# PaddlePaddle/Paddle3D

Measured on NVIDIA H100. Metric: CenterPoint frames/sec @300k pts, 0.075m voxel (0.1m voxel: geometry_01m), 1440x1440x40 grid, higher is better.
Workload: dtype f16x3 (fp16 hi/lo' pairs, f32 accumulation)

## Files before the change

paddle3d_b200/csrc/dense_conv_f16.cu:

```cuda
#include <cuda.h>
#include <cuda_fp16.h>

#include "h16.cuh"
#include "p3d_b200.h"
#include "tc_common.cuh"

namespace p3d {
namespace dcf {

using namespace tc;

constexpr int kTW = 8, kTH = 16;
constexpr int kPitch = kTW + 2;
constexpr int kMaxA = 6, kMaxB = 12;
constexpr int kSmemBudget = (227 - 6) * 1024;
constexpr int kDenseThreads = 384;
constexpr uint32_t kConsumerWarps = 8;
constexpr uint32_t kEpiThreads = 96;

struct Params {
  int B, H, W, Cin;
  int taps, kw, stride, pad;
  int up;
  int oH, oW;
  int tiles_x, tiles_y, n_ntiles;
  int cout;
  int out_H, out_W;
  int out_C, out_c0;
  int relu;
  const uint8_t *packed_w;
  const float *scale, *shift;
  uint8_t *out_h16;
  float *out_nchw;
  int32_t *status;
};

template <int N, int MT, bool HALO>
struct Cfg {
  static constexpr int A_ROWS = HALO ? kPitch * (kTH * MT + 2) : kM * MT;
  static constexpr int A_BYTES = ((A_ROWS * 128 + 1023) / 1024) * 1024;
  static constexpr int B_BYTES = 128 * N;
  static constexpr int B_BLK = 64 * N;
  static constexpr int SP = N + 8;
  static constexpr int STG_WG = MT * 64 * SP;
  static constexpr int STG_BYTES = 2 * STG_WG * 4;
  static constexpr int AVAIL = kSmemBudget - STG_BYTES;
  static constexpr int NA_TAP_RAW = AVAIL / (A_BYTES + B_BYTES);
  static constexpr int NA = HALO ? 2 : (NA_TAP_RAW > kMaxA ? kMaxA : NA_TAP_RAW);
  static constexpr int BUDGET = AVAIL - NA * A_BYTES;
  static constexpr int NB_RAW = BUDGET / B_BYTES;
  static constexpr int NB = NB_RAW > kMaxB ? kMaxB : NB_RAW;
  static constexpr int ACC = MT * N;
  static constexpr int SPU = HALO ? 9 : 1;
  static constexpr int P_REGS = 88, C_REGS = 208;
  static_assert(128 * P_REGS + 256 * C_REGS <= kDenseThreads * 168, "register split");
  static_assert(N == 64 || N == 128, "N tile: 64 or 128");
  static_assert(MT == 1 || MT == 2, "one or two M tiles");
  static_assert(MT * N <= 128, "accumulators: at most 128 registers per thread");
  static_assert(NB >= 3, "weight ring too shallow");
  static_assert(NA >= 2 && NA <= kMaxA, "activation ring depth");
};

__device__ __forceinline__ void tma_tile4d(uint32_t dst, const CUtensorMap *map, int c, int x, int y, int b, uint32_t bar) {
  asm volatile(
      "cp.async.bulk.tensor.4d.shared::cluster.global.tile.mbarrier::complete_tx::bytes [%0], [%1, {%2, %3, %4, %5}], [%6];" ::
          "r"(dst),
      "l"(reinterpret_cast<uint64_t>(map)), "r"(c), "r"(x), "r"(y), "r"(b), "r"(bar)
      : "memory");
}
struct Item {
  int nt, tap0, tx0, ty0, b;
};

enum TraceField {
  kTrItems, kTrCycles,
  kTrAFull, kTrBFull = kTrAFull + 2,
  kTrMma = kTrBFull + 2,
  kTrEpi = kTrMma + 2,
  kTrStageFree = kTrEpi + 2,
  kTrAEmpty = kTrStageFree + 2, kTrBEmpty,
  kTrEwWait, kTrEwBusy,
  kTrFields
};
#ifdef P3D_DENSE_TRACE
constexpr int kTrMaxCtas = 1024;
__device__ unsigned long long g_dense_trace[kTrMaxCtas][kTrFields];
struct Trace {
  unsigned long long sum[kTrFields] = {};
  __device__ __forceinline__ long long now() const { return clock64(); }
  __device__ __forceinline__ void add(int f, long long t0) { sum[f] += static_cast<unsigned long long>(clock64() - t0); }
  __device__ __forceinline__ void count(int f, unsigned long long v) { sum[f] += v; }
  __device__ void flush(int cw) const {
#pragma unroll
    for (int f = 0; f < kTrFields; ++f) {
      const int dst = f >= kTrAFull && f < kTrAEmpty ? f + cw : f;
      if (sum[f]) atomicAdd(&g_dense_trace[blockIdx.x % kTrMaxCtas][dst], sum[f]);
    }
  }
};
#else
struct Trace {
  __device__ __forceinline__ long long now() const { return 0; }
  __device__ __forceinline__ void add(int, long long) {}
  __device__ __forceinline__ void count(int, unsigned long long) {}
  __device__ __forceinline__ void flush(int) const {}
};
#endif
__device__ __forceinline__ Item decode(long long idx, const Params &p, int th) {
  Item it;
  long long q = blockIdx.x + idx * gridDim.x;
  it.nt = static_cast<int>(q % p.n_ntiles);
  q /= p.n_ntiles;
  it.tap0 = 0;
  if (p.up > 1) {
    const int up2 = p.up * p.up;
    it.tap0 = static_cast<int>(q % up2);
    q /= up2;
  }
  it.tx0 = static_cast<int>(q % p.tiles_x) * kTW;
  q /= p.tiles_x;
  it.ty0 = static_cast<int>(q % p.tiles_y) * th;
  it.b = static_cast<int>(q / p.tiles_y);
  return it;
}

template <int N, int MT>
__device__ __forceinline__ void epilogue_warps(const Params &p, const float *stg, unsigned long long *staged,
                                               unsigned long long *freed, long long n_items, int th, int et) {
  constexpr int SP = N + 8, ROWS = MT * 64;
  const int ew = et >> 5, lane = et & 31;
  bool ovf = false;
  Trace tr;
  for (long long idx = 0; idx < n_items; ++idx) {
    const Item im = decode(idx, p, th);
    const int dy = p.up > 1 ? im.tap0 / p.up : 0, dx = p.up > 1 ? im.tap0 % p.up : 0;
    for (int c = 0; c < 2; ++c) {
      long long t0 = tr.now();
      mbar_wait(smem_u32(staged + c), static_cast<uint32_t>(idx & 1));
      tr.add(kTrEwWait, t0);
      t0 = tr.now();
      const float *st = stg + c * ROWS * SP;
      auto pixel = [&](int r, int &Y, int &X) {
        const int m = c * 64 + (r & 63), iy = im.ty0 + (r >> 6) * kTH + m / kTW, ix = im.tx0 + m % kTW;
        Y = iy * p.up + dy;
        X = ix * p.up + dx;
        return iy < p.oH && ix < p.oW;
      };
      if (p.out_h16) {
        const int r4 = lane >> 3, c4 = (lane & 7) * 4;
        for (int q = 0; q < N / 32; ++q) {
          const int col = q * 32 + c4, ch = im.nt * N + col, oc = p.out_c0 + ch;
          if (ch >= p.cout) continue;
          float sc[4], sh[4];
#pragma unroll
          for (int e = 0; e < 4; ++e) {
            sc[e] = p.scale ? __ldg(p.scale + ch + e) : 1.0f;
            sh[e] = p.shift ? __ldg(p.shift + ch + e) : 0.0f;
          }
#pragma unroll 2
          for (int rq = ew; rq < ROWS / 4; rq += 3) {
            const int r = rq * 4 + r4;
            int Y, X;
            if (!pixel(r, Y, X)) continue;
            const float4 o4 = *reinterpret_cast<const float4 *>(st + r * SP + col);
            float v[4] = {o4.x, o4.y, o4.z, o4.w};
#pragma unroll
            for (int e = 0; e < 4; ++e) {
              v[e] = fmaf(v[e], sc[e], sh[e]);
              if (p.relu) v[e] = fmaxf(v[e], 0.f);
            }
            __half2 h01, l01, h23, l23;
            split_h16x2(v[0], v[1], h01, l01, ovf);
            split_h16x2(v[2], v[3], h23, l23, ovf);
            uint8_t *op = p.out_h16 + ((static_cast<size_t>(im.b) * p.out_H + Y) * p.out_W + X) * (4 * static_cast<size_t>(p.out_C)) +
                          (oc / 32) * 128 + (oc % 32) * 2;
            *reinterpret_cast<uint2 *>(op) = make_uint2(*reinterpret_cast<const uint32_t *>(&h01), *reinterpret_cast<const uint32_t *>(&h23));
            *reinterpret_cast<uint2 *>(op + 64) = make_uint2(*reinterpret_cast<const uint32_t *>(&l01), *reinterpret_cast<const uint32_t *>(&l23));
          }
        }
      }
      if (p.out_nchw) {
        const int px = lane & 7, cc = lane >> 3;
        for (int u = ew; u < (ROWS / 8) * (N / 4); u += 3) {
          const int r = (u % (ROWS / 8)) * 8 + px, col = (u / (ROWS / 8)) * 4 + cc, ch = im.nt * N + col;
          int Y, X;
          if (ch >= p.cout || !pixel(r, Y, X)) continue;
          const float sc = p.scale ? __ldg(p.scale + ch) : 1.0f, sh = p.shift ? __ldg(p.shift + ch) : 0.0f;
          float v = fmaf(st[r * SP + col], sc, sh);
          if (p.relu) v = fmaxf(v, 0.f);
          p.out_nchw[((static_cast<size_t>(im.b) * p.cout + ch) * p.out_H + Y) * p.out_W + X] = v;
        }
      }
      mbar_arrive(smem_u32(freed + c));
      tr.add(kTrEwBusy, t0);
    }
  }
  if (ovf && p.status) atomicOr(p.status, 1);
  if (et == 0) tr.flush(0);
}

template <int N, int MT, bool HALO>
__global__ void __launch_bounds__(kDenseThreads, 1)
    dense_conv_f16_kernel(const __grid_constant__ CUtensorMap in_map, const Params p) {
  using C = Cfg<N, MT, HALO>;
  constexpr int TH = kTH * MT;
  constexpr int H = N / 2;
  asm volatile("griddepcontrol.launch_dependents;" ::: "memory");
  asm volatile("griddepcontrol.wait;" ::: "memory");
  const int up2 = p.up * p.up;
  const long long n_total = static_cast<long long>(p.B) * p.tiles_y * p.tiles_x * p.n_ntiles * (p.up > 1 ? up2 : 1);
  if (static_cast<long long>(blockIdx.x) >= n_total) return;
  const long long n_items = (n_total - blockIdx.x + gridDim.x - 1) / gridDim.x;

  extern __shared__ __align__(1024) uint8_t smem_raw[];
  uint8_t *smem = reinterpret_cast<uint8_t *>((reinterpret_cast<uintptr_t>(smem_raw) + 1023) & ~uintptr_t(1023));
  __shared__ __align__(8) unsigned long long s_bar[2 * kMaxA + 2 * kMaxB + 4];
  constexpr int kAF = 0, kAE = kMaxA, kBF = 2 * kMaxA, kBE = 2 * kMaxA + kMaxB, kSS = 2 * kMaxA + 2 * kMaxB, kSF = kSS + 2;

  const int tid = threadIdx.x, wg = tid >> 7, wtid = tid & 127;
  if (tid == 0) {
    for (int s = 0; s < C::NA; ++s) {
      mbar_init(smem_u32(&s_bar[kAF + s]), 1);
      mbar_init(smem_u32(&s_bar[kAE + s]), kConsumerWarps);
    }
    for (int s = 0; s < C::NB; ++s) {
      mbar_init(smem_u32(&s_bar[kBF + s]), 1);
      mbar_init(smem_u32(&s_bar[kBE + s]), kConsumerWarps);
    }
    for (int c = 0; c < 2; ++c) {
      mbar_init(smem_u32(&s_bar[kSS + c]), 128);
      mbar_init(smem_u32(&s_bar[kSF + c]), kEpiThreads);
    }
    fence_mbar_init();
  }
  __syncthreads();
  const uint32_t a_ring = smem_u32(smem);
  const uint32_t b_ring = a_ring + C::NA * C::A_BYTES;
  float *const stg = reinterpret_cast<float *>(smem + C::NA * C::A_BYTES + C::NB * C::B_BYTES);
  const int G = p.Cin / 32;
  const int taps_item = p.up > 1 ? 1 : p.taps;
  const int units_item = HALO ? G : taps_item * G;

  if (wg == 0) {
    asm volatile("setmaxnreg.dec.sync.aligned.u32 %0;" ::"n"(C::P_REGS));
    if (tid >= 32) {
      epilogue_warps<N, MT>(p, stg, s_bar + kSS, s_bar + kSF, n_items, TH, tid - 32);
      return;
    }
    if (tid != 0) return;
    uint32_t a_slot = 0, a_ph = 0, b_slot = 0, b_ph = 0;
    Trace tr;
    for (long long idx = 0; idx < n_items; ++idx) {
      const Item im = decode(idx, p, TH);
      const uint8_t *w_tile = p.packed_w + static_cast<size_t>(im.nt) * p.taps * (p.Cin / 16) * C::B_BLK;
      int dy = 0, dx = 0;
      for (int tu = 0; tu < (HALO ? 1 : taps_item); ++tu) {
        const int tap = p.up > 1 ? im.tap0 : tu;
        for (int g = 0; g < G; ++g) {
          const uint32_t abar = smem_u32(&s_bar[kAF + a_slot]), a_dst = a_ring + a_slot * C::A_BYTES;
          const long long t0 = tr.now();
          mbar_wait(smem_u32(&s_bar[kAE + a_slot]), a_ph ^ 1u);
          tr.add(kTrAEmpty, t0);
          mbar_arrive_expect_tx(abar, static_cast<uint32_t>(C::A_ROWS * 128));
          if (HALO) {
            tma_tile4d(a_dst, &in_map, g * 64, im.tx0 - 1, im.ty0 - 1, im.b, abar);
          } else {
            const int x = im.tx0 * p.stride - p.pad + dx, y = im.ty0 * p.stride - p.pad + dy;
            tma_tile4d(a_dst, &in_map, g * 64, x, y, im.b, abar);
          }
          if (++a_slot == C::NA) a_slot = 0, a_ph ^= 1u;
          for (int t = 0; t < C::SPU; ++t) {
            const uint32_t bbar = smem_u32(&s_bar[kBF + b_slot]);
            const long long t1 = tr.now();
            mbar_wait(smem_u32(&s_bar[kBE + b_slot]), b_ph ^ 1u);
            tr.add(kTrBEmpty, t1);
            mbar_arrive_expect_tx(bbar, static_cast<uint32_t>(C::B_BYTES));
            bulk_g2s(b_ring + b_slot * C::B_BYTES, w_tile + (static_cast<size_t>(HALO ? t : tap) * (p.Cin / 16) + 2 * g) * C::B_BLK,
                     static_cast<uint32_t>(C::B_BYTES), bbar);
            if (++b_slot == C::NB) b_slot = 0, b_ph ^= 1u;
          }
        }
        if (++dx == p.kw) dx = 0, ++dy;
      }
    }
    tr.flush(0);
    return;
  }

  asm volatile("setmaxnreg.inc.sync.aligned.u32 %0;" ::"n"(C::C_REGS));
  const int cw = wg - 1;
  const bool warp_leader = (tid & 31) == 0;
  auto release = [&](int base, uint32_t slot) {
    if (warp_leader) mbar_arrive(smem_u32(&s_bar[base + slot]));
  };
  uint32_t a_slot = 0, a_ph = 0, b_slot = 0, b_ph = 0;
  float acc[C::ACC];
  Trace tr;
  const long long t_start = tr.now();
  for (long long idx = 0; idx < n_items; ++idx) {
#pragma unroll
    for (int i = 0; i < C::ACC; ++i) acc[i] = 0.f;
    uint32_t prev_b = 0;
    int prev_a = -1;
    bool pending = false;
    for (int ua = 0; ua < units_item; ++ua) {
      long long t0 = tr.now();
      mbar_wait(smem_u32(&s_bar[kAF + a_slot]), a_ph);
      tr.add(kTrAFull, t0);
      const uint32_t a_base = a_ring + a_slot * C::A_BYTES;
      for (int t = 0; t < C::SPU; ++t) {
        t0 = tr.now();
        mbar_wait(smem_u32(&s_bar[kBF + b_slot]), b_ph);
        tr.add(kTrBFull, t0);
        const uint32_t b_base = b_ring + b_slot * C::B_BYTES;
        wg_fence();
#pragma unroll
        for (int kb = 0; kb < 2; ++kb) {
          const uint32_t bk = b_base + static_cast<uint32_t>(kb * C::B_BLK);
          const uint64_t dbh = smem_desc(bk, 2 * N * 16, 128), dbl = smem_desc(bk + N * 16, 2 * N * 16, 128);
#pragma unroll
          for (int mt = 0; mt < MT; ++mt) {
            uint32_t a0, sbo;
            if (HALO) {
              a0 = a_base + static_cast<uint32_t>(((mt * kTH + cw * 8 + t / 3) * kPitch + t % 3) * 128);
              sbo = kPitch * 128;
            } else {
              a0 = a_base + static_cast<uint32_t>((mt * kM + cw * 64) * 128);
              sbo = 1024;
            }
            const uint64_t dah = desc_sw128(a0 + kb * 32, sbo), dal = desc_sw128(a0 + (2 + kb) * 32, sbo);
            float *d = acc + mt * N;
            wg::mma_f16<N>(d, dah, dbh, 1u);
            wg::mma_f16<N>(d + H, dah, dbl, 1u);
            wg::mma_f16<N>(d + H, dal, dbh, 1u);
          }
        }
        wg_commit();
        t0 = tr.now();
        wg_wait<1>();
        tr.add(kTrMma, t0);
        if (pending) {
          release(kBE, prev_b);
          if (prev_a >= 0) release(kAE, static_cast<uint32_t>(prev_a));
        }
        pending = true;
        prev_b = b_slot;
        prev_a = t == C::SPU - 1 ? static_cast<int>(a_slot) : -1;
        if (++b_slot == C::NB) b_slot = 0, b_ph ^= 1u;
      }
      if (++a_slot == C::NA) a_slot = 0, a_ph ^= 1u;
    }
    long long t0 = tr.now();
    wg_wait<0>();
    tr.add(kTrMma, t0);
    t0 = tr.now();
    release(kBE, prev_b);
    release(kAE, static_cast<uint32_t>(prev_a));
    wg_fence_acc<C::ACC>(acc);
    tr.add(kTrEpi, t0);
    t0 = tr.now();
    if (idx > 0) mbar_wait(smem_u32(&s_bar[kSF + cw]), static_cast<uint32_t>((idx - 1) & 1));
    tr.add(kTrStageFree, t0);
    t0 = tr.now();
    float *const st = stg + cw * C::STG_WG;
#pragma unroll
    for (int mt = 0; mt < MT; ++mt) {
#pragma unroll
      for (int i = 0; i < H; i += 2) {
        const int r = mt * 64 + frag_row(i, wtid), c = frag_col(i, wtid);
        *reinterpret_cast<float2 *>(st + r * C::SP + c) =
            make_float2(fmaf(acc[mt * N + H + i], kLoInv, acc[mt * N + i]), fmaf(acc[mt * N + H + i + 1], kLoInv, acc[mt * N + i + 1]));
      }
    }
    mbar_arrive(smem_u32(&s_bar[kSS + cw]));
    tr.add(kTrEpi, t0);
  }
  if (cw == 0) {
    tr.count(kTrItems, static_cast<unsigned long long>(n_items));
    tr.add(kTrCycles, t_start);
  }
  if (wtid == 0) tr.flush(cw);
}

__global__ void __launch_bounds__(256) nchw_to_pixel_h16_kernel(const float *__restrict__ in, int C, long long HW,
                                                                __half *__restrict__ out, int32_t *status) {
  __shared__ float s_t[32][33];
  const int b = blockIdx.z;
  const long long p0 = static_cast<long long>(blockIdx.x) * 32;
  const int c0 = blockIdx.y * 32;
  const int tx = threadIdx.x & 31, ty = threadIdx.x >> 5;
  for (int k = ty; k < 32; k += 8) {
    const int c = c0 + k;
    const long long px = p0 + tx;
    s_t[k][tx] = (c < C && px < HW) ? in[(static_cast<size_t>(b) * C + c) * HW + px] : 0.f;
  }
  __syncthreads();
  bool ovf = false;
  for (int k = ty; k < 32; k += 8) {
    const long long px = p0 + k;
    if (px < HW) {
      __half h, l;
      split_h16(s_t[tx][k], h, l, ovf);
      __half *grp = out + (static_cast<size_t>(b) * HW + px) * (2 * static_cast<size_t>(C)) + static_cast<size_t>(c0) * 2;
      grp[tx] = h;
      grp[32 + tx] = l;
    }
  }
  if (ovf && status) atomicOr(status, 1);
}

__global__ void __launch_bounds__(256) pixel_h16_to_nchw_kernel(const __half *__restrict__ in, int C, long long HW,
                                                                float *__restrict__ out, long long total) {
  const long long q = static_cast<long long>(blockIdx.x) * blockDim.x + threadIdx.x;
  if (q >= total) return;
  const long long px = q % HW;
  const int c = static_cast<int>((q / HW) % C);
  const long long b = q / (HW * C);
  const __half *grp = in + (b * HW + px) * (2 * static_cast<long long>(C)) + (c / 32) * 64;
  out[q] = merge_h16(grp[c % 32], grp[32 + c % 32]);
}

inline int make_image_map(const void *img, int B, int H, int W, int Cin, int stride, int box_x, int box_y, CUtensorMap *map) {
  using Encode = CUresult (*)(CUtensorMap *, CUtensorMapDataType, cuuint32_t, void *, const cuuint64_t *, const cuuint64_t *,
                              const cuuint32_t *, const cuuint32_t *, CUtensorMapInterleave, CUtensorMapSwizzle,
                              CUtensorMapL2promotion, CUtensorMapFloatOOBfill);
  static Encode encode = nullptr;
  if (!encode) {
    void *fn = nullptr;
    cudaDriverEntryPointQueryResult qr;
    if (cudaGetDriverEntryPoint("cuTensorMapEncodeTiled", &fn, cudaEnableDefault, &qr) != cudaSuccess || !fn)
      return P3D_ERR_UNSUPPORTED;
    encode = reinterpret_cast<Encode>(fn);
  }
  const cuuint64_t row = static_cast<cuuint64_t>(4) * Cin;
  const cuuint64_t gdim[4] = {static_cast<cuuint64_t>(2 * Cin), static_cast<cuuint64_t>(W), static_cast<cuuint64_t>(H),
                              static_cast<cuuint64_t>(B)};
  const cuuint64_t gstride[3] = {row, row * W, row * W * H};
  const cuuint32_t box[4] = {64u, static_cast<cuuint32_t>(box_x * stride), static_cast<cuuint32_t>(box_y * stride), 1u};
  const cuuint32_t estride[4] = {1u, static_cast<cuuint32_t>(stride), static_cast<cuuint32_t>(stride), 1u};
  const CUresult r = encode(map, CU_TENSOR_MAP_DATA_TYPE_FLOAT16, 4, const_cast<void *>(img), gdim, gstride, box, estride,
                            CU_TENSOR_MAP_INTERLEAVE_NONE, CU_TENSOR_MAP_SWIZZLE_128B, CU_TENSOR_MAP_L2_PROMOTION_NONE,
                            CU_TENSOR_MAP_FLOAT_OOB_FILL_NONE);
  return r == CUDA_SUCCESS ? P3D_OK : P3D_ERR_INVALID_ARG;
}

template <int N, int MT, bool HALO>
int launch(const CUtensorMap &map, const Params &p, cudaStream_t st) {
  using C = Cfg<N, MT, HALO>;
  const size_t smem = static_cast<size_t>(C::NA) * C::A_BYTES + static_cast<size_t>(C::NB) * C::B_BYTES + C::STG_BYTES + 1024;
  if (smem > static_cast<size_t>(kSmemBudget)) return P3D_ERR_UNSUPPORTED;
  auto kern = dense_conv_f16_kernel<N, MT, HALO>;
  P3D_CUDA_CHECK(cudaFuncSetAttribute(kern, cudaFuncAttributeMaxDynamicSharedMemorySize, static_cast<int>(smem)));
  const long long work = static_cast<long long>(p.B) * p.tiles_y * p.tiles_x * p.n_ntiles * (p.up > 1 ? p.up * p.up : 1);
  cudaLaunchConfig_t cfg = {};
  const long long sms = num_sms();
  cfg.gridDim = dim3(static_cast<unsigned int>(work < sms ? work : sms));
  cfg.blockDim = dim3(kDenseThreads);
  cfg.dynamicSmemBytes = smem;
  cfg.stream = st;
  cudaLaunchAttribute attr[1];
  attr[0].id = cudaLaunchAttributeProgrammaticStreamSerialization;
  attr[0].val.programmaticStreamSerializationAllowed = 1;
  cfg.attrs = attr;
  cfg.numAttrs = 1;
  P3D_CUDA_CHECK(cudaLaunchKernelEx(&cfg, kern, map, p));
  P3D_LAUNCH_CHECK();
  return P3D_OK;
}

namespace out9 {
constexpr int kHT = 16, kOT = 14;
constexpr int kRows = kHT * kHT;
constexpr int kABytes = kRows * 128;
constexpr int kN = 32, kStride = 29;
constexpr int kWBlk = 64 * kN;
constexpr int kPBytes = kRows * kStride * 4;
constexpr int kMaxNA = 5, kNW = 3;
constexpr int kAcc = 2 * kN;

struct Params {
  int B, H, W, G;
  int tiles_x, tiles_y, groups, planes, NA;
  const uint8_t *packed_w;
  const float *bias;
  const int32_t *cin0;
  const int32_t *plane0, *cnt;
  float *out;
};

__global__ void __launch_bounds__(kThreads, 1) head_out9_kernel(const __grid_constant__ CUtensorMap in_map, const Params p) {
  asm volatile("griddepcontrol.launch_dependents;" ::: "memory");
  asm volatile("griddepcontrol.wait;" ::: "memory");
  const long long n_work = static_cast<long long>(p.B) * p.tiles_y * p.tiles_x * p.groups;
  if (static_cast<long long>(blockIdx.x) >= n_work) return;
  extern __shared__ __align__(1024) uint8_t smem_raw[];
  uint8_t *smem = reinterpret_cast<uint8_t *>((reinterpret_cast<uintptr_t>(smem_raw) + 1023) & ~uintptr_t(1023));
  __shared__ __align__(8) unsigned long long s_bar[kMaxNA + kNW];
  constexpr int kAF = 0, kWF = kMaxNA;
  const int tid = threadIdx.x, wg = tid >> 7, wtid = tid & 127;
  const int NA = p.NA, G = p.G;
  const uint32_t w_slot = static_cast<uint32_t>(2 * G * kWBlk);
  if (tid == 0) {
    for (int s = 0; s < NA; ++s) mbar_init(smem_u32(&s_bar[kAF + s]), 1);
    for (int s = 0; s < kNW; ++s) mbar_init(smem_u32(&s_bar[kWF + s]), 1);
    fence_mbar_init();
  }
  const uint32_t a_ring = smem_u32(smem);
  const uint32_t w_ring = a_ring + static_cast<uint32_t>(NA * kABytes);
  float *s_p = reinterpret_cast<float *>(smem + static_cast<size_t>(NA) * kABytes + static_cast<size_t>(kNW) * w_slot);

  auto decode = [&](long long w, int &g, int &tx0, int &ty0, int &b) {
    g = static_cast<int>(w % p.groups);
    long long q = w / p.groups;
    tx0 = static_cast<int>(q % p.tiles_x) * kOT;
    q /= p.tiles_x;
    ty0 = static_cast<int>(q % p.tiles_y) * kOT;
    b = static_cast<int>(q / p.tiles_y);
  };
  const long long n_items = (n_work - blockIdx.x + gridDim.x - 1) / gridDim.x;
  const long long n_steps = n_items * G;
  auto issue_a = [&](long long q) {
    int g, tx0, ty0, b;
    decode(blockIdx.x + (q / G) * gridDim.x, g, tx0, ty0, b);
    const int cg0 = (p.cin0 ? __ldg(p.cin0 + g) : g * G * 32) / 32;
    const uint32_t slot = static_cast<uint32_t>(q % NA), bar = smem_u32(&s_bar[kAF + slot]);
    mbar_arrive_expect_tx(bar, static_cast<uint32_t>(kABytes));
    tma_tile4d(a_ring + slot * kABytes, &in_map, (cg0 + static_cast<int>(q % G)) * 64, tx0 - 1, ty0 - 1, b, bar);
  };
  auto issue_w = [&](long long i) {
    const int g = static_cast<int>((blockIdx.x + i * gridDim.x) % p.groups);
    const uint32_t slot = static_cast<uint32_t>(i % kNW), bar = smem_u32(&s_bar[kWF + slot]);
    mbar_arrive_expect_tx(bar, w_slot);
    bulk_g2s(w_ring + slot * w_slot, p.packed_w + static_cast<size_t>(g) * w_slot, w_slot, bar);
  };

  long long next_a = 0, next_w = 0, q = 0;
  float acc[kAcc];
  for (long long idx = 0; idx < n_items; ++idx) {
    int g, tx0, ty0, b;
    decode(blockIdx.x + idx * gridDim.x, g, tx0, ty0, b);
    const int cnt = __ldg(p.cnt + g), p0 = __ldg(p.plane0 + g);
    const float4 bias = __ldg(reinterpret_cast<const float4 *>(p.bias) + g);
#pragma unroll
    for (int i = 0; i < kAcc; ++i) acc[i] = 0.f;
    const uint32_t ws = static_cast<uint32_t>(idx % kNW);
    for (int k = 0; k < G; ++k, ++q) {
      __syncthreads();
      if (tid == 0) {
        for (; next_a < n_steps && next_a <= q + NA - 1; ++next_a) issue_a(next_a);
        for (; next_w < n_items && (next_w - kNW + 1) * G <= q; ++next_w) issue_w(next_w);
      }
      if (k == 0) mbar_wait(smem_u32(&s_bar[kWF + ws]), static_cast<uint32_t>((idx / kNW) & 1));
      const uint32_t sa = static_cast<uint32_t>(q % NA);
      mbar_wait(smem_u32(&s_bar[kAF + sa]), static_cast<uint32_t>((q / NA) & 1));
      const uint32_t a_base = a_ring + sa * kABytes;
      const uint32_t w_base = w_ring + ws * w_slot;
      wg_fence();
#pragma unroll
      for (int kb = 0; kb < 2; ++kb) {
        const uint32_t bk = w_base + static_cast<uint32_t>((k * 2 + kb) * kWBlk);
        const uint64_t dbh = smem_desc(bk, 2 * kN * 16, 128), dbl = smem_desc(bk + kN * 16, 2 * kN * 16, 128);
#pragma unroll
        for (int mt = 0; mt < 2; ++mt) {
          const uint32_t a0 = a_base + static_cast<uint32_t>((mt * kM + wg * 64) * 128);
          const uint64_t dah = desc_sw128(a0 + kb * 32), dal = desc_sw128(a0 + (2 + kb) * 32);
          float *d = acc + mt * kN;
          wg::mma_f16<kN>(d, dah, dbh, 1u);
          wg::mma_f16<kN>(d + kN / 2, dah, dbl, 1u);
          wg::mma_f16<kN>(d + kN / 2, dal, dbh, 1u);
        }
      }
      wg_commit();
      wg_wait<0>();
    }
    wg_fence_acc<kAcc>(acc);
#pragma unroll
    for (int mt = 0; mt < 2; ++mt) {
#pragma unroll
      for (int i = 0; i < kN / 2; ++i) {
        const int r = mt * kM + wg * 64 + frag_row(i, wtid), c = frag_col(i, wtid);
        if (c < 27) s_p[r * kStride + c] = fmaf(acc[mt * kN + kN / 2 + i], kLoInv, acc[mt * kN + i]);
      }
    }
    __syncthreads();
    for (int o = tid; o < kOT * kOT; o += kThreads) {
      const int oy = o / kOT, ox = o - oy * kOT;
      const int Y = ty0 + oy, X = tx0 + ox;
      if (Y < p.H && X < p.W) {
        float s0 = bias.x, s1 = bias.y, s2 = bias.z;
#pragma unroll
        for (int t = 0; t < 9; ++t) {
          const float *e = s_p + ((oy + t / 3) * kHT + ox + t % 3) * kStride + t * 3;
          s0 += e[0];
          s1 += e[1];
          s2 += e[2];
        }
        float *op = p.out + ((static_cast<size_t>(b) * p.planes + p0) * p.H + Y) * p.W + X;
        const size_t plane = static_cast<size_t>(p.H) * p.W;
        op[0] = s0;
        if (cnt > 1) op[plane] = s1;
        if (cnt > 2) op[2 * plane] = s2;
      }
    }
  }
}
}

}
}

using namespace p3d;

extern "C" int p3d_nchw_to_pixel_h16(const float *in, int B, int C, int H, int W, void *out_h16, int32_t *status_dev,
                                     p3d_stream_t stream) {
  if (!in || !out_h16 || B < 1 || C < 32 || C % 32 || H < 1 || W < 1) return P3D_ERR_INVALID_ARG;
  const long long hw = static_cast<long long>(H) * W;
  dim3 grid(static_cast<unsigned int>((hw + 31) / 32), static_cast<unsigned int>(C / 32), B);
  dcf::nchw_to_pixel_h16_kernel<<<grid, 256, 0, static_cast<cudaStream_t>(stream)>>>(in, C, hw, static_cast<__half *>(out_h16),
                                                                                      status_dev);
  P3D_LAUNCH_CHECK();
  return P3D_OK;
}

extern "C" int p3d_pixel_h16_to_nchw(const void *in_h16, int B, int C, int H, int W, float *out, p3d_stream_t stream) {
  if (!in_h16 || !out || B < 1 || C < 32 || C % 32 || H < 1 || W < 1) return P3D_ERR_INVALID_ARG;
  const long long hw = static_cast<long long>(H) * W, total = hw * C * B;
  dcf::pixel_h16_to_nchw_kernel<<<div_up(total, 256), 256, 0, static_cast<cudaStream_t>(stream)>>>(
      static_cast<const __half *>(in_h16), C, hw, out, total);
  P3D_LAUNCH_CHECK();
  return P3D_OK;
}

#ifdef P3D_DENSE_TRACE
extern "C" int p3d_dense_trace_read(unsigned long long *host, int max_ctas, int reset) {
  const size_t n = static_cast<size_t>(max_ctas < dcf::kTrMaxCtas ? max_ctas : dcf::kTrMaxCtas) * dcf::kTrFields;
  P3D_CUDA_CHECK(cudaDeviceSynchronize());
  if (host) P3D_CUDA_CHECK(cudaMemcpyFromSymbol(host, dcf::g_dense_trace, n * sizeof(unsigned long long)));
  if (reset) {
    void *dev = nullptr;
    P3D_CUDA_CHECK(cudaGetSymbolAddress(&dev, dcf::g_dense_trace));
    P3D_CUDA_CHECK(cudaMemset(dev, 0, sizeof(dcf::g_dense_trace)));
    P3D_CUDA_CHECK(cudaDeviceSynchronize());
  }
  return dcf::kTrFields;
}
#endif

extern "C" size_t p3d_dense_conv2d_f16_packed_weight_bytes(int taps, int Cin, int Cout, int n_tile) {
  if (taps < 1 || Cin < 32 || Cin % 32 || Cout < 1 || (n_tile != 16 && n_tile != 32 && n_tile != 64 && n_tile != 128)) return 0;
  const size_t tiles = static_cast<size_t>((Cout + n_tile - 1) / n_tile);
  return align_up(tiles * taps * Cin * static_cast<size_t>(n_tile) * 4);
}

extern "C" int p3d_dense_conv2d_f16(const void *in_h16, int B, int H, int W, int Cin, const void *packed_weight, int Cout,
                                    int n_tile, int kh, int kw, int stride, int pad, int up, const float *scale,
                                    const float *shift, int relu, void *out_h16, int out_C, int out_c0, float *out_nchw,
                                    int mode, int m_tiles, int32_t *status_dev, p3d_stream_t stream) {
  if (!in_h16 || !packed_weight || (!out_h16 && !out_nchw) || B < 1 || H < 1 || W < 1 || Cout < 1 || (mode != 0 && mode != 1))
    return P3D_ERR_INVALID_ARG;
  if (Cin < 32 || Cin % 32 || (n_tile != 64 && n_tile != 128)) return P3D_ERR_UNSUPPORTED;
  if (up < 1 || (up > 1 && (kh != up || kw != up || stride != up || pad != 0))) return P3D_ERR_UNSUPPORTED;
  if (up == 1 && (kh < 1 || kw < 1 || kh * kw > 32 || stride < 1 || stride > 2 || pad < 0)) return P3D_ERR_UNSUPPORTED;
  if (out_h16 && (Cout % 16 || out_C % 32 || out_c0 % 16 || out_c0 + Cout > out_C)) return P3D_ERR_INVALID_ARG;
  if ((reinterpret_cast<uintptr_t>(in_h16) & 15) || (reinterpret_cast<uintptr_t>(packed_weight) & 15) ||
      (reinterpret_cast<uintptr_t>(out_h16) & 15))
    return P3D_ERR_INVALID_ARG;
  dcf::Params p;
  p.B = B;
  p.H = H;
  p.W = W;
  p.Cin = Cin;
  p.taps = kh * kw;
  p.kw = kw;
  p.up = up;
  p.stride = up > 1 ? 1 : stride;
  p.pad = up > 1 ? 0 : pad;
  p.oH = up > 1 ? H : (H + 2 * pad - kh) / stride + 1;
  p.oW = up > 1 ? W : (W + 2 * pad - kw) / stride + 1;
  if (p.oH < 1 || p.oW < 1) return P3D_ERR_INVALID_ARG;
  p.out_H = up > 1 ? H * up : p.oH;
  p.out_W = up > 1 ? W * up : p.oW;
  p.n_ntiles = (Cout + n_tile - 1) / n_tile;
  p.cout = Cout;
  p.out_C = out_C;
  p.out_c0 = out_c0;
  p.relu = relu;
  p.packed_w = static_cast<const uint8_t *>(packed_weight);
  p.scale = scale;
  p.shift = shift;
  p.out_h16 = static_cast<uint8_t *>(out_h16);
  p.out_nchw = out_nchw;
  p.status = status_dev;
  const bool halo = mode == 0 && up == 1 && kh == 3 && kw == 3 && stride == 1 && pad == 1;
  int mt = m_tiles;
  if (mt != 1 && mt != 2) {
    const long long tx = (p.oW + dcf::kTW - 1) / dcf::kTW, sms = num_sms();
    const long long per_row = static_cast<long long>(B) * tx * p.n_ntiles * (up > 1 ? up * up : 1);
    const long long items1 = per_row * ((p.oH + dcf::kTH - 1) / dcf::kTH), items2 = per_row * ((p.oH + 2 * dcf::kTH - 1) / (2 * dcf::kTH));
    mt = (n_tile <= 64 && 2 * ((items2 + sms - 1) / sms) <= (items1 + sms - 1) / sms) ? 2 : 1;
  }
  if (n_tile > 64) mt = 1;
  p.tiles_x = (p.oW + dcf::kTW - 1) / dcf::kTW;
  p.tiles_y = (p.oH + dcf::kTH * mt - 1) / (dcf::kTH * mt);
  CUtensorMap map;
  const int bx = halo ? dcf::kPitch : dcf::kTW, by = halo ? dcf::kTH * mt + 2 : dcf::kTH * mt;
  const int rc = dcf::make_image_map(in_h16, B, H, W, Cin, p.stride, bx, by, &map);
  if (rc != P3D_OK) return rc;
  cudaStream_t st = static_cast<cudaStream_t>(stream);
  if (n_tile == 128) return halo ? dcf::launch<128, 1, true>(map, p, st) : dcf::launch<128, 1, false>(map, p, st);
  if (mt == 2) return halo ? dcf::launch<64, 2, true>(map, p, st) : dcf::launch<64, 2, false>(map, p, st);
  return halo ? dcf::launch<64, 1, true>(map, p, st) : dcf::launch<64, 1, false>(map, p, st);
}

extern "C" int p3d_head_out_conv_f16(const void *in_h16, int B, int H, int W, int in_C, int Cin, int groups,
                                     const void *packed_weight, const float *bias, const int32_t *cin0_dev,
                                     const int32_t *plane0_dev, const int32_t *cnt_dev, int planes, float *out_nchw,
                                     p3d_stream_t stream) {
  if (!in_h16 || !packed_weight || !bias || !plane0_dev || !cnt_dev || !out_nchw || B < 1 || H < 1 || W < 1 || groups < 1 ||
      planes < 1 || in_C % 32 || Cin > in_C)
    return P3D_ERR_INVALID_ARG;
  if (Cin < 32 || Cin % 32) return P3D_ERR_UNSUPPORTED;
  if ((reinterpret_cast<uintptr_t>(in_h16) & 15) || (reinterpret_cast<uintptr_t>(packed_weight) & 15) ||
      (reinterpret_cast<uintptr_t>(bias) & 15))
    return P3D_ERR_INVALID_ARG;
  namespace o9 = dcf::out9;
  const long long w_ring = static_cast<long long>(o9::kNW) * 2 * (Cin / 32) * o9::kWBlk;
  const long long na = (dcf::kSmemBudget - 1024 - o9::kPBytes - w_ring) / o9::kABytes;
  if (na < 2) return P3D_ERR_UNSUPPORTED;
  o9::Params p;
  p.B = B;
  p.H = H;
  p.W = W;
  p.G = Cin / 32;
  p.tiles_x = (W + o9::kOT - 1) / o9::kOT;
  p.tiles_y = (H + o9::kOT - 1) / o9::kOT;
  p.groups = groups;
  p.planes = planes;
  p.NA = static_cast<int>(na < o9::kMaxNA ? na : o9::kMaxNA);
  p.packed_w = static_cast<const uint8_t *>(packed_weight);
  p.bias = bias;
  p.cin0 = cin0_dev;
  p.plane0 = plane0_dev;
  p.cnt = cnt_dev;
  p.out = out_nchw;
  CUtensorMap map;
  const int rc = dcf::make_image_map(in_h16, B, H, W, in_C, 1, o9::kHT, o9::kHT, &map);
  if (rc != P3D_OK) return rc;
  const size_t smem = static_cast<size_t>(p.NA) * o9::kABytes + static_cast<size_t>(w_ring) + o9::kPBytes + 1024;
  auto kern = o9::head_out9_kernel;
  P3D_CUDA_CHECK(cudaFuncSetAttribute(kern, cudaFuncAttributeMaxDynamicSharedMemorySize, static_cast<int>(smem)));
  const long long work = static_cast<long long>(B) * p.tiles_y * p.tiles_x * groups;
  cudaLaunchConfig_t cfg = {};
  const long long sms = num_sms();
  cfg.gridDim = dim3(static_cast<unsigned int>(work < sms ? work : sms));
  cfg.blockDim = dim3(tc::kThreads);
  cfg.dynamicSmemBytes = smem;
  cfg.stream = static_cast<cudaStream_t>(stream);
  cudaLaunchAttribute attr[1];
  attr[0].id = cudaLaunchAttributeProgrammaticStreamSerialization;
  attr[0].val.programmaticStreamSerializationAllowed = 1;
  cfg.attrs = attr;
  cfg.numAttrs = 1;
  P3D_CUDA_CHECK(cudaLaunchKernelEx(&cfg, kern, map, p));
  P3D_LAUNCH_CHECK();
  return P3D_OK;
}
```

Measured before the change: 389.9.

## Move fp16 pair epilogue into consumer warps and write output via TMA stores

For the fp16 hi/lo output path, consumer warps now apply scale/shift/ReLU and split into fp16 pairs directly from registers into a swizzled shared tile. The epilogue warps then issue TMA tensor stores (4D, or 5D for upsampled outputs) instead of doing per-element float staging and scalar stores. A scalar fallback remains for partial channel blocks. This removes the fp32 staging round trip and the scalar global writes. The cost is extra work and a named barrier in the consumer warps, plus an additional tensor map encode on the host.

Measured after the change: 404.7 (median of 6 runs). 1.04x the previous value.

```diff
diff --git a/paddle3d_b200/csrc/dense_conv_f16.cu b/paddle3d_b200/csrc/dense_conv_f16.cu
--- a/paddle3d_b200/csrc/dense_conv_f16.cu
+++ b/paddle3d_b200/csrc/dense_conv_f16.cu
@@ -44,6 +44,8 @@
   static constexpr int SP = N + 8;
   static constexpr int STG_WG = MT * 64 * SP;
   static constexpr int STG_BYTES = 2 * STG_WG * 4;
+  static constexpr int PAIR_BLK = 64 * 128, PAIR_BYTES = MT * (N / 32) * PAIR_BLK;
+  static_assert(PAIR_BYTES + 2 * 2 * N * 4 <= STG_WG * 4 && STG_WG * 4 % 1024 == 0, "pair tile inside the staging tile");
   static constexpr int AVAIL = kSmemBudget - STG_BYTES;
   static constexpr int NA_TAP_RAW = AVAIL / (A_BYTES + B_BYTES);
   static constexpr int NA = HALO ? 2 : (NA_TAP_RAW > kMaxA ? kMaxA : NA_TAP_RAW);
@@ -68,6 +70,29 @@
       "l"(reinterpret_cast<uint64_t>(map)), "r"(c), "r"(x), "r"(y), "r"(b), "r"(bar)
       : "memory");
 }
+__device__ __forceinline__ void tma_store4d(const CUtensorMap *map, uint32_t src, int c, int x, int y, int b) {
+  asm volatile("cp.async.bulk.tensor.4d.global.shared::cta.bulk_group [%0, {%2, %3, %4, %5}], [%1];" ::"l"(
+                   reinterpret_cast<uint64_t>(map)),
+               "r"(src), "r"(c), "r"(x), "r"(y), "r"(b)
+               : "memory");
+}
+__device__ __forceinline__ void tma_store5d(const CUtensorMap *map, uint32_t src, int c, int d1, int d2, int d3, int d4) {
+  asm volatile("cp.async.bulk.tensor.5d.global.shared::cta.bulk_group [%0, {%2, %3, %4, %5, %6}], [%1];" ::"l"(
+                   reinterpret_cast<uint64_t>(map)),
+               "r"(src), "r"(c), "r"(d1), "r"(d2), "r"(d3), "r"(d4)
+               : "memory");
+}
+__device__ __forceinline__ void st_shared_u32(uint32_t addr, uint32_t v) {
+  asm volatile("st.shared.b32 [%0], %1;" ::"r"(addr), "r"(v));
+}
+__device__ __forceinline__ float2 ld_shared_f2(uint32_t addr) {
+  float2 v;
+  asm("ld.shared.v2.f32 {%0, %1}, [%2];" : "=f"(v.x), "=f"(v.y) : "r"(addr));
+  return v;
+}
+__device__ __forceinline__ void bulk_commit() { asm volatile("cp.async.bulk.commit_group;" ::: "memory"); }
+__device__ __forceinline__ void bulk_wait_read() { asm volatile("cp.async.bulk.wait_group.read 0;" ::: "memory"); }
+__device__ __forceinline__ void bulk_wait_all() { asm volatile("cp.async.bulk.wait_group 0;" ::: "memory"); }
 struct Item {
   int nt, tap0, tx0, ty0, b;
 };
@@ -199,9 +224,69 @@
   if (et == 0) tr.flush(0);
 }
 
+template <int N, int MT>
+__device__ __forceinline__ void epilogue_pairs(const Params &p, const CUtensorMap *out_map, const uint8_t *tiles, int tile_bytes,
+                                               unsigned long long *staged, unsigned long long *freed, long long n_items,
+                                               int th, int et) {
+  constexpr int NQ = N / 32, BLK = 64 * 128;
+  const bool lead = et == 0;
+  const bool whole = p.out_c0 % 32 == 0;
+  Trace tr;
+  for (long long idx = 0; idx < n_items; ++idx) {
+    const Item im = decode(idx, p, th);
+    const int dy = p.up > 1 ? im.tap0 / p.up : 0, dx = p.up > 1 ? im.tap0 % p.up : 0;
+    for (int c = 0; c < 2; ++c) {
+      long long t0 = tr.now();
+      mbar_wait(smem_u32(staged + c), static_cast<uint32_t>(idx & 1));
+      tr.add(kTrEwWait, t0);
+      t0 = tr.now();
+      for (int blk = 0; blk < MT * NQ; ++blk) {
+        const int ch0 = im.nt * N + (blk % NQ) * 32, iy0 = im.ty0 + (blk / NQ) * kTH + c * 8;
+        if (ch0 >= p.cout) continue;
+        const uint8_t *src = tiles + c * tile_bytes + blk * BLK;
+        if (whole && ch0 + 32 <= p.cout) {
+          if (!lead) continue;
+          const int hc = 2 * (p.out_c0 + ch0);
+          if (p.up == 1) {
+            tma_store4d(out_map, smem_u32(src), hc, im.tx0, iy0, im.b);
+          } else {
+            for (int y = 0; y < 8 && iy0 + y < p.oH; ++y)
+              tma_store5d(out_map, smem_u32(src + y * 1024), hc, dx, im.tx0, dy, im.b * p.oH + iy0 + y);
+          }
+          continue;
+        }
+        for (int u = et; u < 128; u += kEpiThreads) {
+          const int r = u >> 1, h = u & 1, iy = iy0 + (r >> 3), ix = im.tx0 + (r & 7);
+          if (ch0 + 16 * h >= p.cout || iy >= p.oH || ix >= p.oW) continue;
+          const int oc = p.out_c0 + ch0 + 16 * h, Y = iy * p.up + dy, X = ix * p.up + dx;
+          uint8_t *op = p.out_h16 + ((static_cast<size_t>(im.b) * p.out_H + Y) * p.out_W + X) * (4 * static_cast<size_t>(p.out_C)) +
+                        (oc / 32) * 128 + (oc % 32) * 2;
+          const uint8_t *row = src + r * 128;
+#pragma unroll
+          for (int k = 0; k < 2; ++k) {
+            *reinterpret_cast<uint4 *>(op + 16 * k) = *reinterpret_cast<const uint4 *>(row + (((2 * h + k) ^ (r & 7)) << 4));
+            *reinterpret_cast<uint4 *>(op + 64 + 16 * k) = *reinterpret_cast<const uint4 *>(row + (((4 + 2 * h + k) ^ (r & 7)) << 4));
+          }
+        }
+      }
+      if (lead) {
+        bulk_commit();
+        bulk_wait_read();
+      }
+      mbar_arrive(smem_u32(freed + c));
+      tr.add(kTrEwBusy, t0);
+    }
+  }
+  if (lead) {
+    bulk_wait_all();
+    tr.flush(0);
+  }
+}
+
 template <int N, int MT, bool HALO>
 __global__ void __launch_bounds__(kDenseThreads, 1)
-    dense_conv_f16_kernel(const __grid_constant__ CUtensorMap in_map, const Params p) {
+    dense_conv_f16_kernel(const __grid_constant__ CUtensorMap in_map, const __grid_constant__ CUtensorMap out_map,
+                          const Params p) {
   using C = Cfg<N, MT, HALO>;
   constexpr int TH = kTH * MT;
   constexpr int H = N / 2;
@@ -237,6 +322,7 @@
   const uint32_t a_ring = smem_u32(smem);
   const uint32_t b_ring = a_ring + C::NA * C::A_BYTES;
   float *const stg = reinterpret_cast<float *>(smem + C::NA * C::A_BYTES + C::NB * C::B_BYTES);
+  const bool pairs = p.out_nchw == nullptr;
   const int G = p.Cin / 32;
   const int taps_item = p.up > 1 ? 1 : p.taps;
   const int units_item = HALO ? G : taps_item * G;
@@ -244,7 +330,11 @@
   if (wg == 0) {
     asm volatile("setmaxnreg.dec.sync.aligned.u32 %0;" ::"n"(C::P_REGS));
     if (tid >= 32) {
-      epilogue_warps<N, MT>(p, stg, s_bar + kSS, s_bar + kSF, n_items, TH, tid - 32);
+      if (pairs)
+        epilogue_pairs<N, MT>(p, &out_map, reinterpret_cast<const uint8_t *>(stg), C::STG_WG * 4, s_bar + kSS, s_bar + kSF,
+                              n_items, TH, tid - 32);
+      else
+        epilogue_warps<N, MT>(p, stg, s_bar + kSS, s_bar + kSF, n_items, TH, tid - 32);
       return;
     }
     if (tid != 0) return;
@@ -295,11 +385,21 @@
   };
   uint32_t a_slot = 0, a_ph = 0, b_slot = 0, b_ph = 0;
   float acc[C::ACC];
+  bool ovf = false;
   Trace tr;
   const long long t_start = tr.now();
   for (long long idx = 0; idx < n_items; ++idx) {
 #pragma unroll
     for (int i = 0; i < C::ACC; ++i) acc[i] = 0.f;
+    const Item im = decode(idx, p, TH);
+    const uint32_t ss = smem_u32(stg) + cw * C::STG_WG * 4 + C::PAIR_BYTES + static_cast<uint32_t>(idx & 1) * 2 * N * 4;
+    if (pairs) {
+      for (int c = wtid; c < 2 * N; c += 128) {
+        const int ch = im.nt * N + c % N;
+        const float *src = c < N ? p.scale : p.shift;
+        st_shared_u32(ss + c * 4, __float_as_uint(ch < p.cout && src ? __ldg(src + ch) : (c < N ? 1.0f : 0.0f)));
+      }
+    }
     uint32_t prev_b = 0;
     int prev_a = -1;
     bool pending = false;
@@ -362,19 +462,59 @@
     if (idx > 0) mbar_wait(smem_u32(&s_bar[kSF + cw]), static_cast<uint32_t>((idx - 1) & 1));
     tr.add(kTrStageFree, t0);
     t0 = tr.now();
-    float *const st = stg + cw * C::STG_WG;
-#pragma unroll
-    for (int mt = 0; mt < MT; ++mt) {
-#pragma unroll
-      for (int i = 0; i < H; i += 2) {
-        const int r = mt * 64 + frag_row(i, wtid), c = frag_col(i, wtid);
-        *reinterpret_cast<float2 *>(st + r * C::SP + c) =
-            make_float2(fmaf(acc[mt * N + H + i], kLoInv, acc[mt * N + i]), fmaf(acc[mt * N + H + i + 1], kLoInv, acc[mt * N + i + 1]));
+    if (pairs) {
+      const int lane = wtid & 31, key = lane >> 2;
+      const uint32_t row = smem_u32(stg) + cw * C::STG_WG * 4 + ((wtid >> 5) * 16 + key) * 128 + (lane & 3) * 4;
+      uint32_t a_hi[4], a_lo[4];
+#pragma unroll
+      for (int jj = 0; jj < 4; ++jj) a_hi[jj] = row + ((jj ^ key) << 4), a_lo[jj] = row + (((4 + jj) ^ key) << 4);
+      uint32_t after_bar;
+      asm volatile("bar.sync %1, 128;\n\tmov.u32 %0, 0;" : "=r"(after_bar) : "r"(1 + cw) : "memory");
+      const uint32_t sc_col = ss + after_bar + (lane & 3) * 8;
+      bool o[MT][2] = {};
+#pragma unroll
+      for (int j = 0; j < N / 8; ++j) {
+        const float2 sc = ld_shared_f2(sc_col + j * 32), sh = ld_shared_f2(sc_col + (N + j * 8) * 4);
+        const float sc0 = sc.x, sc1 = sc.y, sh0 = sh.x, sh1 = sh.y;
+#pragma unroll
+        for (int mt = 0; mt < MT; ++mt) {
+#pragma unroll
+          for (int h = 0; h < 2; ++h) {
+            const int i = j * 4 + h * 2;
+            float v0 = fmaf(acc[mt * N + H + i], kLoInv, acc[mt * N + i]);
+            float v1 = fmaf(acc[mt * N + H + i + 1], kLoInv, acc[mt * N + i + 1]);
+            v0 = fmaf(v0, sc0, sh0);
+            v1 = fmaf(v1, sc1, sh1);
+            if (p.relu) v0 = fmaxf(v0, 0.f), v1 = fmaxf(v1, 0.f);
+            __half2 hi, lo;
+            split_h16x2(v0, v1, hi, lo, o[mt][h]);
+            const uint32_t off = (mt * (N / 32) + j / 4) * C::PAIR_BLK + h * 8 * 128;
+            st_shared_u32(a_hi[j & 3] + off, *reinterpret_cast<const uint32_t *>(&hi));
+            st_shared_u32(a_lo[j & 3] + off, *reinterpret_cast<const uint32_t *>(&lo));
+          }
+        }
+      }
+      const int iy = im.ty0 + cw * 8 + (wtid >> 5) * 2, ix = im.tx0 + key;
+#pragma unroll
+      for (int mt = 0; mt < MT; ++mt)
+        ovf |= ix < p.oW && ((o[mt][0] && iy + mt * kTH < p.oH) || (o[mt][1] && iy + mt * kTH + 1 < p.oH));
+      fence_proxy_async();
+    } else {
+      float *const st = stg + cw * C::STG_WG;
+#pragma unroll
+      for (int mt = 0; mt < MT; ++mt) {
+#pragma unroll
+        for (int i = 0; i < H; i += 2) {
+          const int r = mt * 64 + frag_row(i, wtid), c = frag_col(i, wtid);
+          *reinterpret_cast<float2 *>(st + r * C::SP + c) =
+              make_float2(fmaf(acc[mt * N + H + i], kLoInv, acc[mt * N + i]), fmaf(acc[mt * N + H + i + 1], kLoInv, acc[mt * N + i + 1]));
+        }
       }
     }
     mbar_arrive(smem_u32(&s_bar[kSS + cw]));
     tr.add(kTrEpi, t0);
   }
+  if (ovf && p.status) atomicOr(p.status, 1);
   if (cw == 0) {
     tr.count(kTrItems, static_cast<unsigned long long>(n_items));
     tr.add(kTrCycles, t_start);
@@ -420,18 +560,23 @@
   out[q] = merge_h16(grp[c % 32], grp[32 + c % 32]);
 }
 
-inline int make_image_map(const void *img, int B, int H, int W, int Cin, int stride, int box_x, int box_y, CUtensorMap *map) {
-  using Encode = CUresult (*)(CUtensorMap *, CUtensorMapDataType, cuuint32_t, void *, const cuuint64_t *, const cuuint64_t *,
-                              const cuuint32_t *, const cuuint32_t *, CUtensorMapInterleave, CUtensorMapSwizzle,
-                              CUtensorMapL2promotion, CUtensorMapFloatOOBfill);
+using Encode = CUresult (*)(CUtensorMap *, CUtensorMapDataType, cuuint32_t, void *, const cuuint64_t *, const cuuint64_t *,
+                            const cuuint32_t *, const cuuint32_t *, CUtensorMapInterleave, CUtensorMapSwizzle,
+                            CUtensorMapL2promotion, CUtensorMapFloatOOBfill);
+inline Encode tensor_map_encoder() {
   static Encode encode = nullptr;
   if (!encode) {
     void *fn = nullptr;
     cudaDriverEntryPointQueryResult qr;
-    if (cudaGetDriverEntryPoint("cuTensorMapEncodeTiled", &fn, cudaEnableDefault, &qr) != cudaSuccess || !fn)
-      return P3D_ERR_UNSUPPORTED;
+    if (cudaGetDriverEntryPoint("cuTensorMapEncodeTiled", &fn, cudaEnableDefault, &qr) != cudaSuccess || !fn) return nullptr;
     encode = reinterpret_cast<Encode>(fn);
   }
+  return encode;
+}
+
+inline int make_image_map(const void *img, int B, int H, int W, int Cin, int stride, int box_x, int box_y, CUtensorMap *map) {
+  const Encode encode = tensor_map_encoder();
+  if (!encode) return P3D_ERR_UNSUPPORTED;
   const cuuint64_t row = static_cast<cuuint64_t>(4) * Cin;
   const cuuint64_t gdim[4] = {static_cast<cuuint64_t>(2 * Cin), static_cast<cuuint64_t>(W), static_cast<cuuint64_t>(H),
                               static_cast<cuuint64_t>(B)};
@@ -444,8 +589,32 @@
   return r == CUDA_SUCCESS ? P3D_OK : P3D_ERR_INVALID_ARG;
 }
 
+inline int make_out_map(void *img, int B, int H, int W, int out_C, int up, CUtensorMap *map) {
+  const Encode encode = tensor_map_encoder();
+  if (!encode) return P3D_ERR_UNSUPPORTED;
+  const cuuint64_t row = static_cast<cuuint64_t>(4) * out_C;
+  CUresult r;
+  if (up == 1) {
+    const cuuint64_t gdim[4] = {static_cast<cuuint64_t>(2 * out_C), static_cast<cuuint64_t>(W), static_cast<cuuint64_t>(H),
+                                static_cast<cuuint64_t>(B)};
+    const cuuint64_t gstride[3] = {row, row * W, row * W * H};
+    const cuuint32_t box[4] = {64u, static_cast<cuuint32_t>(kTW), 8u, 1u}, estride[4] = {1u, 1u, 1u, 1u};
+    r = encode(map, CU_TENSOR_MAP_DATA_TYPE_FLOAT16, 4, img, gdim, gstride, box, estride, CU_TENSOR_MAP_INTERLEAVE_NONE,
+               CU_TENSOR_MAP_SWIZZLE_128B, CU_TENSOR_MAP_L2_PROMOTION_NONE, CU_TENSOR_MAP_FLOAT_OOB_FILL_NONE);
+  } else {
+    const cuuint64_t u = static_cast<cuuint64_t>(up), ow = u * W;
+    const cuuint64_t gdim[5] = {static_cast<cuuint64_t>(2 * out_C), u, static_cast<cuuint64_t>(W), u,
+                                static_cast<cuuint64_t>(B) * H};
+    const cuuint64_t gstride[4] = {row, row * u, row * ow, row * ow * u};
+    const cuuint32_t box[5] = {64u, 1u, static_cast<cuuint32_t>(kTW), 1u, 1u}, estride[5] = {1u, 1u, 1u, 1u, 1u};
+    r = encode(map, CU_TENSOR_MAP_DATA_TYPE_FLOAT16, 5, img, gdim, gstride, box, estride, CU_TENSOR_MAP_INTERLEAVE_NONE,
+               CU_TENSOR_MAP_SWIZZLE_128B, CU_TENSOR_MAP_L2_PROMOTION_NONE, CU_TENSOR_MAP_FLOAT_OOB_FILL_NONE);
+  }
+  return r == CUDA_SUCCESS ? P3D_OK : P3D_ERR_INVALID_ARG;
+}
+
 template <int N, int MT, bool HALO>
-int launch(const CUtensorMap &map, const Params &p, cudaStream_t st) {
+int launch(const CUtensorMap &map, const CUtensorMap &out_map, const Params &p, cudaStream_t st) {
   using C = Cfg<N, MT, HALO>;
   const size_t smem = static_cast<size_t>(C::NA) * C::A_BYTES + static_cast<size_t>(C::NB) * C::B_BYTES + C::STG_BYTES + 1024;
   if (smem > static_cast<size_t>(kSmemBudget)) return P3D_ERR_UNSUPPORTED;
@@ -463,7 +632,7 @@
   attr[0].val.programmaticStreamSerializationAllowed = 1;
   cfg.attrs = attr;
   cfg.numAttrs = 1;
-  P3D_CUDA_CHECK(cudaLaunchKernelEx(&cfg, kern, map, p));
+  P3D_CUDA_CHECK(cudaLaunchKernelEx(&cfg, kern, map, out_map, p));
   P3D_LAUNCH_CHECK();
   return P3D_OK;
 }
@@ -704,12 +873,14 @@
   p.tiles_y = (p.oH + dcf::kTH * mt - 1) / (dcf::kTH * mt);
   CUtensorMap map;
   const int bx = halo ? dcf::kPitch : dcf::kTW, by = halo ? dcf::kTH * mt + 2 : dcf::kTH * mt;
-  const int rc = dcf::make_image_map(in_h16, B, H, W, Cin, p.stride, bx, by, &map);
+  int rc = dcf::make_image_map(in_h16, B, H, W, Cin, p.stride, bx, by, &map);
   if (rc != P3D_OK) return rc;
+  CUtensorMap omap = {};
+  if (!out_nchw && (rc = dcf::make_out_map(out_h16, B, p.oH, p.oW, out_C, up, &omap)) != P3D_OK) return rc;
   cudaStream_t st = static_cast<cudaStream_t>(stream);
-  if (n_tile == 128) return halo ? dcf::launch<128, 1, true>(map, p, st) : dcf::launch<128, 1, false>(map, p, st);
-  if (mt == 2) return halo ? dcf::launch<64, 2, true>(map, p, st) : dcf::launch<64, 2, false>(map, p, st);
-  return halo ? dcf::launch<64, 1, true>(map, p, st) : dcf::launch<64, 1, false>(map, p, st);
+  if (n_tile == 128) return halo ? dcf::launch<128, 1, true>(map, omap, p, st) : dcf::launch<128, 1, false>(map, omap, p, st);
+  if (mt == 2) return halo ? dcf::launch<64, 2, true>(map, omap, p, st) : dcf::launch<64, 2, false>(map, omap, p, st);
+  return halo ? dcf::launch<64, 1, true>(map, omap, p, st) : dcf::launch<64, 1, false>(map, omap, p, st);
 }
 
 extern "C" int p3d_head_out_conv_f16(const void *in_h16, int B, int H, int W, int in_C, int Cin, int groups,
```
